# Luka140/paig_reproduction

Measured on AMD Instinct MI355X. Metric: video-seqs/sec (train step) spring_color B=100 @ 1/2/4/8 MI355X, higher is better.
Workload: dtype fp32; 1 GPU; spring_color PhysicsNet train step (get_batch gather+fwd+loss+bwd+allreduce+RMSprop), B=100/rank, 32x32x3, seq_len 50 (4 in / 6 pred / 40 extrap); global_batch=100, seq_len=50, parallelism=dp1, conv_math=split, split_graph=False, optimizer_in_graph=True, byte_targets=True, dataset_seqs=800

## Files before the change

### include/paig_hip.h

```cpp
#ifndef PAIG_HIP_H
#define PAIG_HIP_H
#include <stddef.h>

#ifdef __cplusplus
extern "C" {
#endif

#define PAIG_ABI_VERSION 9
const char* paig_last_error(void);
int paig_abi_version(void);
int paig_f16_range_status(int clear);

int paig_conv2d_fwd(const float* in, long long in_fs, int in_grp, long long in_gs, float* out, long long out_fs,
                    const float* aux, long long aux_fs, const float* w, const float* bias, int F, int Cin, int Cout,
                    int H, int W, int ks, int flags, void* stream);
#define PAIG_XMAX_SLOTS 2048
int paig_conv2d_fwd_ex(const float* in, long long in_fs, int in_grp, long long in_gs, float* out, long long out_fs,
                       const float* aux, long long aux_fs, const float* w, const float* bias, int F, int Cin,
                       int Cout, int H, int W, int ks, int flags, float* xmax, int xmax_n, void* stream);
int paig_conv2d_fwd_pw(const float* in, long long in_fs, int in_grp, long long in_gs, float* out, long long out_fs,
                       const float* aux, long long aux_fs, const float* w, const float* bias, int F, int Cin,
                       int Cout, int H, int W, int ks, int flags, float* xmax, int xmax_n, float* pool_out,
                       long long pool_fs, const void* wprep, void* stream);
int paig_conv2d_fwd_pwc(const float* in, long long in_fs, int in_grp, long long in_gs, float* out, long long out_fs,
                        const float* aux, long long aux_fs, const float* w, const float* bias, int F, int Cin,
                        int Cout, int H, int W, int ks, int flags, float* xmax, int xmax_n, float* pool_out,
                        long long pool_fs, unsigned char* pool_code, long long pool_code_fs, const void* wprep,
                        void* stream);
long long paig_conv_wprep_size(int cin, int cout, int ks);
int paig_conv_wprep(int n, const float* const* w, const int* cin, const int* cout, const int* ks, const int* dg,
                    void* const* out, void* stream);
int paig_conv_wprep_defer(int n, const float* const* w, const int* cin, const int* cout, const int* ks, const int* dg,
                          void* const* out, void* stream);
int paig_conv_wprep_flush(void* stream);
int paig_debug_fwd_block_cap(int cap);
int paig_conv2d_mfma_supported(int what, int Cin, int Cout, int H, int W, int ks, int flags);
int paig_conv2d_wgrad(const float* x, long long x_fs, int x_grp, long long x_gs, const float* dy, long long dy_fs,
                      float* slab, int nblk_max, int* nblk_out, int F, int Cin, int Cout, int H, int W, int ks,
                      int flags, void* stream);
int paig_conv2d_wgrad_ex(const float* x, long long x_fs, int x_grp, long long x_gs, const float* dy, long long dy_fs,
                         float* slab, int nblk_max, int* nblk_out, int F, int Cin, int Cout, int H, int W, int ks,
                         int flags, const float* xmax, int xmax_n, void* stream);
int paig_conv2d_bwd_supported(int Cin, int Cout, int H, int W, int ks, int flags);
int paig_conv2d_bwd(const float* x, long long x_fs, int x_grp, long long x_gs, const float* dy, long long dy_fs,
                    float* dx, long long dx_fs, const float* aux, long long aux_fs, const float* w, float* slab,
                    int nblk_max, int* nblk_out, int F, int Cin, int Cout, int H, int W, int ks, int flags,
                    const float* xmax, int xmax_n, const float* dpool, long long dpool_fs,
                    const unsigned char* pcode, long long pcode_fs, const void* wprep, void* stream);

size_t paig_unet_workspace(int net, int F, int H, int K, int math);
// ... 49 lines not shown
int paig_mask_softmax_bwd(const float* logits, const float* x, long long x_fs, int x_grp, long long x_gs,
                          const float* masks, const float* dobjs, float* dlogits, int F, int K, int C, int H, int W,
                          int flags, void* stream);
int paig_head_mask_blocks(int F, int H, int W);
int paig_head_mask_fwd(const float* x12, const float* w, const float* b, const float* x, long long x_fs, int x_grp,
                       long long x_gs, float* masks, float* objs, int F, int K, int H, int W, void* stream);
int paig_head_mask_bwd(const float* x12, const float* w, const float* b, const float* x, long long x_fs, int x_grp,
                       long long x_gs, const float* masks, const float* dobjs, float* dx12, float* slab, int F, int K,
                       int H, int W, void* stream);
int paig_head_mask_fwd_ex(const float* xl, const float* w, const float* b, const float* x, long long x_fs, int x_grp,
                          long long x_gs, float* masks, float* objs, float* pobjs, int F, int K, int CI, int H, int W,
                          int flags, void* stream);
int paig_head_mask_bwd_ex(const float* xl, const float* w, const float* b, const float* x, long long x_fs, int x_grp,
                          long long x_gs, const float* masks, const float* dobjs, float* dxl, float* slab, int F, int K,
                          int CI, int H, int W, int flags, void* stream);
int paig_pos_head_fwd(const float* h3, float* pos, int N, int K, float half, void* stream);
int paig_pos_head_bwd(const float* h3, const float* dpos, float* dh3, int N, int K, float half, void* stream);

size_t paig_gemm_workspace(int M, int N, int K);
int paig_gemm_defer_epilogue(int on);
int paig_gemm_flush(void* stream);
int paig_gemm(int ta, int tb, int M, int N, int K, float alpha, const float* A, long long lda, const float* B,
              long long ldb, float beta, float* C, long long ldc, const float* bias, int act, int auxm,
              const float* aux, long long ldaux, float* rowsum, float* ws, size_t ws_floats, void* stream);
int paig_gemm_ex(int ta, int tb, int M, int N, int K, float alpha, const float* A, long long lda, const float* B,
                 long long ldb, float beta, float* C, long long ldc, const float* bias, int act, int auxm,
                 const float* aux, long long ldaux, float* rowsum, float* ws, size_t ws_floats, int math,
                 void* stream);
size_t paig_gemm_parts_size(int M, int N, int K, int math);
int paig_gemm_parts(int ta, int tb, int M, int N, int K, const float* A, long long lda, const float* B,
                    long long ldb, float* part, size_t part_floats, int math, void* stream);
size_t paig_colsum_workspace(int M, int N);
int paig_colsum(const float* X, int M, int N, long long ld, float* out, int accumulate, float* ws, void* stream);
int paig_slab_reduce(const float* slab, int nblk, long long ld, int len, float* out, int accumulate, void* stream);
int paig_slab_reduce_multi(int ntask, const float* const* src, const int* nblk, const int* len, float* const* dst,
                           int accumulate, void* stream);
int paig_axpby(const float* x, float* y, long long n, float a, float b, void* stream);

int paig_vfn_fwd(const float* W1, const float* b1, const float* W2, const float* b2, float* hout, float* y,
                 float* ypost, int P, void* stream);
int paig_vfn_bwd_blocks(int P);
int paig_vfn_bwd(const float* d, const float* y, int sig, const float* h, const float* W2, float* dW1, float* db1,
                 float* dW2, float* db2, float* part, int P, void* stream);
// ... 159 lines not shown
```

### paig_reproduction_amd/_lib.py

```python
import ctypes
import os

import torch

_HERE = os.path.dirname(os.path.abspath(__file__))
LIB_PATH = os.path.join(_HERE, "libpaig_hip.so")
XMAX_SLOTS = 2048

AB_PATH = os.environ.get("PAIG_AB_LIB")
ABI_VERSION = 9

P = ctypes.c_void_p
I = ctypes.c_int
LL = ctypes.c_longlong
F32 = ctypes.c_float
F64 = ctypes.c_double
SZ = ctypes.c_size_t

SIGNATURES = {
    "paig_last_error": (ctypes.c_char_p, []),
    "paig_abi_version": (I, []),
    "paig_f16_range_status": (I, [I]),
    "paig_conv2d_fwd": (I, [P, LL, I, LL, P, LL, P, LL, P, P, I, I, I, I, I, I, I, P]),
    "paig_conv2d_wgrad": (I, [P, LL, I, LL, P, LL, P, I, P, I, I, I, I, I, I, I, P]),
    "paig_conv2d_fwd_ex": (I, [P, LL, I, LL, P, LL, P, LL, P, P, I, I, I, I, I, I, I, P, I, P]),
    "paig_conv2d_fwd_pw": (I, [P, LL, I, LL, P, LL, P, LL, P, P, I, I, I, I, I, I, I, P, I, P, LL, P, P]),
    "paig_conv_wprep_size": (LL, [I, I, I]),
    "paig_conv_wprep": (I, [I, P, P, P, P, P, P, P]),
    "paig_conv_wprep_defer": (I, [I, P, P, P, P, P, P, P]),
    "paig_conv_wprep_flush": (I, [P]),
    "paig_conv2d_wgrad_ex": (I, [P, LL, I, LL, P, LL, P, I, P, I, I, I, I, I, I, I, P, I, P]),
    "paig_conv2d_wgrad_pf": (I, [P, LL, I, LL, P, LL, P, LL, P, LL, P, I, P, I, I, I, I, I, I, I, P, I, P]),
    "paig_conv2d_mfma_supported": (I, [I, I, I, I, I, I, I]),
    "paig_debug_fwd_block_cap": (I, [I]),
    "paig_conv2d_bwd_supported": (I, [I, I, I, I, I, I]),
    "paig_conv2d_bwd": (I, [P, LL, I, LL, P, LL, P, LL, P, LL, P, P, I, P, I, I, I, I, I, I, I, P, I, P, LL, P, LL,
                            P, P]),
    "paig_conv2d_fwd_pwc": (I, [P, LL, I, LL, P, LL, P, LL, P, P, I, I, I, I, I, I, I, P, I, P, LL, P, LL, P, P]),
    "paig_gather_u8_f32": (I, [P, P, P, I, LL, P]),
    "paig_gather_u8_f32_ex": (I, [P, P, P, I, LL, LL, P, P]),
    "paig_velmlp_fwd": (I, [P, I, I, I, I, P, P, P, P, P, P, P, P, P, P, P]),
    "paig_velmlp_vfn_fwd": (I, [P, I, I, I, I, P, P, P, P, P, P, P, P, P, P, I, P, P, P, P, P, P, P, P, P]),
    "paig_velmlp_bwd_blocks": (I, [I]),
    "paig_velmlp_slab_len": (I, [I]),
    "paig_velmlp_bwd": (I, [P, P, P, P, P, P, P, P, P, I, I, P]),
    "paig_head_fwd": (I, [P, P, P, P, P, I, I, I, F32, P]),
    "paig_dense_tail_fwd": (I, [P, I, P, P, P, P, P, P, P, P, P, P, I, I, I, F32, P]),
    "paig_head_l2_bwd": (I, [P, P, P, P, P, P, I, I, I, F32, P, P, I, I, I, I, P, P, P, I, P, P, P, P, P, P, P, P, P,
                             P, P, P]),
# ... 17 lines not shown
    "paig_unet_query": (I, [I, I, I]),
    "paig_unet_fwd_ex": (I, [I, I, I, I, I, I, P, LL, I, LL, P, P, P, P, P, P, SZ, P, P, P]),
    "paig_unet_bwd_ex": (I, [I, I, I, I, I, I, P, LL, I, LL, P, P, P, P, I, P, P, P, P, P, P, SZ, P, P, P]),
    "paig_maxpool2_fwd": (I, [P, LL, P, LL, I, I, I, I, P]),
    "paig_maxpool2_fwd_codes": (I, [P, LL, P, LL, P, LL, I, I, I, I, P]),
    "paig_maxpool2_bwd_relu": (I, [P, LL, P, LL, P, LL, I, I, I, I, P]),
    "paig_upsample2_fwd": (I, [P, LL, P, LL, I, I, I, I, I, I, P]),
    "paig_upsample2_bwd": (I, [P, LL, P, LL, P, LL, I, I, I, I, I, I, I, P]),
    "paig_mask_softmax_fwd": (I, [P, P, LL, I, LL, P, P, P, I, I, I, I, I, P]),
    "paig_mask_softmax_bwd": (I, [P, P, LL, I, LL, P, P, P, I, I, I, I, I, I, P]),
    "paig_head_mask_blocks": (I, [I, I, I]),
    "paig_head_mask_fwd": (I, [P, P, P, P, LL, I, LL, P, P, I, I, I, I, P]),
    "paig_head_mask_bwd": (I, [P, P, P, P, LL, I, LL, P, P, P, P, I, I, I, I, P]),
    "paig_head_mask_fwd_ex": (I, [P, P, P, P, LL, I, LL, P, P, P, I, I, I, I, I, I, P]),
    "paig_head_mask_bwd_ex": (I, [P, P, P, P, LL, I, LL, P, P, P, P, I, I, I, I, I, I, P]),
    "paig_pos_head_fwd": (I, [P, P, I, I, F32, P]),
    "paig_pos_head_bwd": (I, [P, P, P, I, I, F32, P]),
    "paig_gemm_workspace": (SZ, [I, I, I]),
    "paig_gemm_parts_size": (SZ, [I, I, I, I]),
    "paig_gemm_parts": (I, [I, I, I, I, I, P, LL, P, LL, P, SZ, I, P]),
    "paig_gemm_defer_epilogue": (I, [I]),
    "paig_gemm_flush": (I, [P]),
    "paig_gemm": (I, [I, I, I, I, I, F32, P, LL, P, LL, F32, P, LL, P, I, I, P, LL, P, P, SZ, P]),
    "paig_gemm_ex": (I, [I, I, I, I, I, F32, P, LL, P, LL, F32, P, LL, P, I, I, P, LL, P, P, SZ, I, P]),
    "paig_colsum_workspace": (SZ, [I, I]),
    "paig_colsum": (I, [P, I, I, LL, P, I, P, P]),
    "paig_slab_reduce": (I, [P, I, LL, I, P, I, P]),
    "paig_slab_reduce_multi": (I, [I, P, P, P, P, I, P]),
    "paig_axpby": (I, [P, P, LL, F32, F32, P]),
    "paig_vfn_fwd": (I, [P, P, P, P, P, P, P, I, P]),
# ... 28 lines not shown
    "paig_loss_bwd": (I, [P, P, P, F32, P, P, I, I, I, I, P]),
    "paig_frame_sse": (I, [P, LL, I, LL, P, LL, I, LL, P, I, I, P]),
    "paig_frame_sse_bwd": (I, [P, LL, I, LL, P, LL, I, LL, P, P, I, I, P]),
    "paig_synth_integrate": (I, [I, P, P, LL, I, I, I, F64, F64, F64, F64, F64, P, P, P]),
    "paig_synth_raster": (I, [P, P, LL, I, I, I, F64, P, P, P]),
    "paig_rmsprop_f32": (I, [P, P, P, LL, F32, F32, F32, P]),
    "paig_rmsprop_f64": (I, [P, P, P, LL, F64, F64, F64, P]),
    "paig_rmsprop_mixed": (I, [P, P, P, LL, P, P, P, LL, F64, F64, F64, P]),
    "paig_adam_f32": (I, [P, P, P, P, LL, F32, F32, F32, F32, F32, F32, P]),
    "paig_adam_f64": (I, [P, P, P, P, LL, F64, F64, F64, F64, F64, F64, P]),
    "paig_sgd_f32": (I, [P, P, P, LL, F32, F32, I, P]),
    "paig_sgd_f64": (I, [P, P, P, LL, F64, F64, I, P]),
}

_QUERY = {"paig_last_error", "paig_abi_version", "paig_f16_range_status", "paig_conv2d_mfma_supported",
          "paig_debug_fwd_block_cap",
          "paig_conv2d_bwd_supported", "paig_velmlp_bwd_blocks",
          "paig_velmlp_slab_len", "paig_head_bwd_blocks", "paig_head_l2_bwd_blocks", "paig_head_mask_blocks", "paig_conv_wprep_size", "paig_gemm_workspace", "paig_colsum_workspace",
          "paig_gemm_parts_size", "paig_gemm_parts", "paig_unet_workspace", "paig_unet_workspace_ex",
          "paig_unet_buffer", "paig_unet_query", "paig_localiser_workspace",
          "paig_velmlp_rollout_bwd_workspace",
          "paig_vfn_bwd_blocks", "paig_rollout_bwd_blocks", "paig_decoder_bwd_blocks", "paig_decoder_slab_len",
          "paig_decoder_bwd_scratch"}


class PaigError(RuntimeError):
    pass


class _Lib:
    def __init__(self, path=LIB_PATH):
# ... 61 lines not shown
```

### paig_reproduction_amd/csrc/conv_split.hip

```cpp
#include "split_common.h"

#ifndef PAIG_FWD_AUXP
#define PAIG_FWD_AUXP 1
#endif

namespace {


constexpr bool sfwd_sla(bool UPS, int PM, int H, int W, int ups_bytes, int lo_bytes) {
  return UPS && PM == 0 && H * W >= 4096 && ups_bytes <= lo_bytes;
}
constexpr int sfwd_lds(int CIN, int H, int W, int KS, bool UPS, int PM, int tpxm, int ntb) {
  const int CC = rup(CIN, 8) / 8, PS = CC % 2 == 0 ? CC + 1 : CC;
  const int NS = ceil_div(KS * KS * CC, 4);
  const int FPT = H * W <= tpxm ? tpxm / (H * W) : 1;
  const int RT = H * W <= tpxm ? H : rows_fit(H, W, tpxm);
  const int TWPX = W + 2 * (KS / 2);
  const int RP = W == 8 ? to_mod16(TWPX * PS, 8) : TWPX * PS;
  const int img = FPT * (RT + KS - 1) * RP * 8, wimg = NS * ntb * 64 * 8;
  const int ups = UPS ? up_window_floats(CIN, FPT, RT, W) * 4 : 0;
  return (img + wimg) * 2 * (PM == 2 ? 1 : 2) + (sfwd_sla(UPS, PM, H, W, ups, img * 2) ? 0 : ups);
}
constexpr int sfwd_vgprs(int CIN, int H, int W, int KS, bool UPS, int tpxm, int ntb) {
  const int CC = rup(CIN, 8) / 8, NS = ceil_div(KS * KS * CC, 4);
// ... 1323 lines not shown
  int blk0[WPREP_MAX + 1];
  int n;
};
constexpr int WPREP_T = 256;

__device__ __forceinline__ int wprep_hdr_entries(int cout) { return (cout + 15) / 16 * 16 * 4 / 16; }

#ifndef PAIG_WPREP_S
#define PAIG_WPREP_S 8
#endif
constexpr int WPREP_S = PAIG_WPREP_S;
__device__ __forceinline__ void conv_wprep_body(const WPrepJobs& jobs, int bid) {
  int q = 0;
  while (q + 1 < jobs.n && bid >= jobs.blk0[q + 1]) ++q;
  const WPrepJob jb = jobs.j[q];
  if (jb.dg == 2) {
    __shared__ float T[32][33];
    const int bl = bid - jobs.blk0[q], tx = (bl % ((jb.cin + 31) / 32)) * 32,
              ty = (bl / ((jb.cin + 31) / 32)) * 32, c = threadIdx.x & 31, r = threadIdx.x >> 5;
    for (int y = r; y < 32; y += WPREP_T / 32)
      if (ty + y < jb.cout && tx + c < jb.cin) T[y][c] = jb.w[(long long)(ty + y) * jb.cin + tx + c];
    __syncthreads();
    float* o = reinterpret_cast<float*>(jb.out);
    for (int y = r; y < 32; y += WPREP_T / 32)
      if (tx + y < jb.cin && ty + c < jb.cout) o[(long long)(tx + y) * jb.cout + ty + c] = T[c][y];
    return;
  }
  const int KK = jb.ks * jb.ks, CC = (jb.cin + 7) / 8, KC = KK * CC, NTT = (jb.cout + 15) / 16, NS = (KC + 3) / 4;
  const int NSC = (NS + WPREP_S - 1) / WPREP_S;
  const int bl = bid - jobs.blk0[q], nt = bl / NSC, s0 = (bl % NSC) * WPREP_S;
  const int tid = threadIdx.x;
  auto wv = [&](int kc, int j, int co) {
    float v = 0.f;
    if (kc < KC && co < jb.cout) {
      const int tap = kc / CC, ci = (kc % CC) * 8 + j;
      if (ci < jb.cin) v = jb.dg ? jb.w[(ci * jb.cout + co) * KK + (KK - 1 - tap)] : jb.w[(co * jb.cin + ci) * KK + tap];
    }
    return v;
  };
  __shared__ float red[WPREP_T];
  __shared__ int ex[16];
  const int cl = tid & 15, co = nt * 16 + cl;
  float m = 0.f;
#pragma unroll 8
  for (int i = tid >> 4; i < KC * 8; i += WPREP_T / 16) m = fmaxf(m, fabsf(wv(i >> 3, i & 7, co)));
  red[tid] = m;
  __syncthreads();
  if (tid < 16) {
    float mm = 0.f;
    for (int r = 0; r < WPREP_T / 16; ++r) mm = fmaxf(mm, red[r * 16 + tid]);
    ex[tid] = f16_scale_exp_v(mm);
    if (s0 == 0) reinterpret_cast<int*>(jb.out)[nt * 16 + tid] = ex[tid];
  }
  __syncthreads();
  const int HDR = wprep_hdr_entries(jb.cout), ENT = NS * NTT * 64;
  short* img = reinterpret_cast<short*>(jb.out + HDR);
// ... 27 lines not shown

WPrepJobs g_wpend{};
int g_wpend_blocks = 0;
int wprep_build(WPrepJobs& jobs, int n, const float* const* w, const int* cin, const int* cout, const int* ks,
                const int* dg, void* const* out, int* blocks_out) {
  jobs = WPrepJobs{};
  jobs.n = n;
  int blocks = 0;
  for (int q = 0; q < n; ++q) {
    PAIG_REQUIRE(w[q] && out[q] && cin[q] > 0 && cout[q] > 0 && ks[q] > 0, "conv_wprep: job %d", q);
    PAIG_REQUIRE(((uintptr_t)out[q] & 15) == 0, "conv_wprep: job %d output not 16-byte aligned", q);
    jobs.j[q] = WPrepJob{w[q], static_cast<s16x8*>(out[q]), cin[q], cout[q], ks[q], dg[q]};
    jobs.blk0[q] = blocks;
    if (dg[q] == 2) {
      blocks += (cin[q] + 31) / 32 * ((cout[q] + 31) / 32);
      continue;
    }
    const int NS = (ks[q] * ks[q] * ((cin[q] + 7) / 8) + 3) / 4;
    blocks += (cout[q] + 15) / 16 * ((NS + WPREP_S - 1) / WPREP_S);
  }
  jobs.blk0[n] = blocks;
  *blocks_out = blocks;
  return 0;
}
int wprep_flush(hipStream_t st) {
  if (!g_wpend_blocks) return 0;
  const int nb = g_wpend_blocks;
  g_wpend_blocks = 0;
  hipLaunchKernelGGL(conv_wprep_k, dim3(nb), dim3(WPREP_T), 0, st, g_wpend);
  PAIG_CHECK_LAUNCH();
// ... 275 lines not shown
}

extern "C" {

int paig_debug_fwd_block_cap(int cap) {
  const int prev = g_fwd_block_cap;
  g_fwd_block_cap = cap > 0 ? cap : 0;
  return prev;
}

long long paig_conv_wprep_size(int cin, int cout, int ks) {
  const int KC = ks * ks * ((cin + 7) / 8), NS = (KC + 3) / 4, NTT = (cout + 15) / 16;
  return 2ll * NS * NTT * 64 * 8 + (long long)NTT * 16 * 2;
}

int paig_conv_wprep(int n, const float* const* w, const int* cin, const int* cout, const int* ks, const int* dg,
                    void* const* out, void* stream) {
  if (int rc = wprep_flush((hipStream_t)stream)) return rc;
  for (int b = 0; b < n; b += WPREP_MAX) {
    WPrepJobs jobs;
    int blocks = 0;
    const int m = n - b < WPREP_MAX ? n - b : WPREP_MAX;
    if (int rc = wprep_build(jobs, m, w + b, cin + b, cout + b, ks + b, dg + b, out + b, &blocks)) return rc;
    hipLaunchKernelGGL(conv_wprep_k, dim3(blocks), dim3(WPREP_T), 0, (hipStream_t)stream, jobs);
    PAIG_CHECK_LAUNCH();
  }
  return 0;
}

int paig_conv_wprep_defer(int n, const float* const* w, const int* cin, const int* cout, const int* ks, const int* dg,
// ... 15 lines not shown
```

### paig_reproduction_amd/csrc/gemm.hip

```cpp
#include "common.h"

#include <algorithm>
#include <cstdlib>

namespace {

constexpr int BM = 64, BN = 64, BK = 32;
constexpr int LDRK = BK + 2;
constexpr int LDKR = 64 + 16;
constexpr int IMG = (BK * LDKR > 64 * LDRK ? BK * LDKR : 64 * LDRK);

typedef float f32x4 __attribute__((ext_vector_type(4)));

__device__ __attribute__((aligned(16))) float zero16[4];

template <bool KCONTIG>
struct Tile {
  f32x4 v[2];
  __device__ __forceinline__ void load(const float* __restrict__ p, long long ld, int r0, int k0, int R, int K,
                                       bool vec, int tid) {
#pragma unroll
    for (int e = 0; e < 2; ++e) {
      int r, k;
      if (KCONTIG) { r = (tid >> 3) + 32 * e; k = (tid & 7) * 4; }
// ... 839 lines not shown
    if (tile == 1) PAIG_W((gemm_split_w_k<TA, TB, PM_, true, 64, 256>)); \
    else if (tile == 2) PAIG_W((gemm_split_w_k<TA, TB, PM_, true, 256, 64>)); \
    else PAIG_S(PM_);                                                   \
  } while (0)
  if (math == 1) PAIG_S(1);
  else if (math == 2) PAIG_S(2);
  else if (math == 3) PAIG_SW(3);
  else if (math == 4) PAIG_SW(4);
  else if (math == 5) PAIG_S(5);
  else if (math == 6) PAIG_SW(6);
  else PAIG_L((gemm_k<TA, TB>));
#undef PAIG_SW
#undef PAIG_S
#undef PAIG_W
#undef PAIG_L
}

}

static PendEpi make_epi(int M, int N, int S, const float* part, float* C, long long ldc, float beta, const float* bias,
                        int act, int auxm, const float* aux, long long ldaux, const float* rowpart, float* rowsum) {
  const bool v4 = N % 4 == 0 && vec_ok(C, ldc) && (!bias || (uintptr_t)bias % 16 == 0) &&
                  (!aux || auxm == AUX_NONE || vec_ok(aux, ldaux)) && (uintptr_t)part % 16 == 0 &&
                  (long long)S * M * N < (1ll << 31) && (long long)M * ldc < (1ll << 31) &&
                  (long long)M * ldaux < (1ll << 31) &&
                  (long long)M * N >= (1 << 19);
  return PendEpi{M, N, S, part, C, ldc, beta, bias, act, auxm, aux, ldaux, rowpart, rowsum, v4 ? 1 : 0};
}
static void launch_epi(const PendEpi& e, hipStream_t st) {
  long long n_el = (e.v4 ? (long long)e.M * e.N / 4 : (long long)e.M * e.N) + (e.rowsum ? e.M : 0);
// ... 129 lines not shown
  else PAIG_G(false, false);
#undef PAIG_G
  PAIG_CHECK_LAUNCH();
  if (S > 1) {
    const PendEpi e = make_epi(M, N, S, part, C, ldc, beta, bias, act, auxm, aux, ldaux, rowpart, rowsum);
    if (defer) {
      g_pend = e;
    } else {
      launch_epi(e, st);
      PAIG_CHECK_LAUNCH();
    }
  }
  return 0;
}

}

PAIG_F16_RANGE_ACCESSOR(paig_f16_range_gemm)
```

### paig_reproduction_amd/csrc/unet_ops.hip

```cpp
#include "common.h"

#define PAIG_MAX_SLAB_TASKS 32

namespace {

template <typename I>
__global__ void maxpool_fwd_k(FView x, FViewW y, int F, int C, int H, int W) {
  const int Ho = H / 2, Wo = W / 2;
  const I n = (I)F * C * Ho * Wo;
  for (I i = blockIdx.x * (I)blockDim.x + threadIdx.x; i < n; i += (I)gridDim.x * blockDim.x) {
    int j = i % Wo;
    I t = i / Wo;
    int ii = t % Ho;
    t /= Ho;
    int c = t % C;
    int f = (int)(t / C);
    const float* xp = x.frame(f) + ((long long)c * H + 2 * ii) * W + 2 * j;
    float m = xp[0];
    float v = xp[1];
    if (v > m || v != v) m = v;
    v = xp[W];
    if (v > m || v != v) m = v;
    v = xp[W + 1];
    if (v > m || v != v) m = v;
// ... 541 lines not shown
            pa[k][c].x += o[1];
            pa[k][c].y += o[2];
            pa[k][c].y += o[3];
          }
      }
    }
#pragma unroll
    for (int k = 0; k < K; ++k)
#pragma unroll
      for (int c = 0; c < 3; ++c)
        *reinterpret_cast<float2*>(pobjs + ((long long)k * F + f) * 3 * HW4 + (long long)c * HW4 + py * W2 + 2 * u) =
            make_float2(pa[k][c].x * 0.25f, pa[k][c].y * 0.25f);
  }
}

template <int K, int CI, bool RELU, bool POOL>
__global__ void __launch_bounds__(256) head_mask_bwd_k(const float* __restrict__ xl, const float* __restrict__ w,
                                                       const float* __restrict__ b, FView x,
                                                       const float* __restrict__ masks, const float* __restrict__ dobjs,
                                                       float* __restrict__ dxl, float* __restrict__ slab, int F, int H,
                                                       int W) {
  constexpr int NW = K * CI + K;
  const int HW = H * W, W2 = W / 2, HW4 = (H / 2) * W2;
  const int DHW = POOL ? HW4 : HW;
  const int Q = HW / 4;
  const long long n = (long long)F * Q;
  float acc[NW];
#pragma unroll
  for (int t = 0; t < NW; ++t) acc[t] = 0.f;
  for (long long i = blockIdx.x * (long long)blockDim.x + threadIdx.x; i < n; i += (long long)gridDim.x * blockDim.x) {
    const int p = (int)(i % Q) * 4;
    const int f = (int)(i / Q);
    const int pq = POOL ? ((p / W) >> 1) * W2 + ((p % W) >> 1) : p;
    m4 hv[CI];
#pragma unroll
    for (int c = 0; c < CI; ++c) hv[c] = *reinterpret_cast<const m4*>(xl + ((long long)f * CI + c) * HW + p);
    const float* xp = x.frame(f);
    m4 xv[3];
#pragma unroll
    for (int c = 0; c < 3; ++c) xv[c] = *reinterpret_cast<const m4*>(xp + c * HW + p);
    m4 dm[K], mk[K];
    m4 dot = m4{0.f, 0.f, 0.f, 0.f};
#pragma unroll
    for (int k = 0; k < K; ++k) {
      m4 a = m4{0.f, 0.f, 0.f, 0.f};
#pragma unroll
      for (int c = 0; c < 3; ++c) {
        const float* dp = dobjs + ((long long)k * F + f) * 3 * DHW + (long long)c * DHW + pq;
        m4 d;
        if constexpr (POOL) {
          const float2 dq = *reinterpret_cast<const float2*>(dp);
          d = m4{dq.x, dq.x, dq.y, dq.y} * 0.25f;
        } else {
          d = *reinterpret_cast<const m4*>(dp);
        }
#pragma unroll
        for (int j = 0; j < 4; ++j) a[j] = fmaf(d[j], xv[c][j], a[j]);
      }
      dm[k] = a;
      mk[k] = *reinterpret_cast<const m4*>(masks + ((long long)f * (K + 1) + k) * HW + p);
#pragma unroll
      for (int j = 0; j < 4; ++j) dot[j] = fmaf(mk[k][j], a[j], dot[j]);
// ... 394 lines not shown
                       logits, FView{x, x_fs, x_gs, x_grp}, masks, dobjs, dlogits, F, K, C, H, W, flags);
  PAIG_CHECK_LAUNCH();
  return 0;
}

static bool head_mask_ok(const void* a, const void* b, const void* c, const void* d, const void* e, long long x_fs,
                         long long x_gs, int K, int H, int W) {
  return (H * W) % 4 == 0 && (K == 2 || K == 3) && x_fs % 4 == 0 && x_gs % 4 == 0 &&
         ((uintptr_t)a | (uintptr_t)b | (uintptr_t)c | (uintptr_t)d | (uintptr_t)e) % 16 == 0;
}
static bool head_mask_kind(int CI, int flags, int H, int W, const void* pobjs) {
  if (CI == 8 && flags == 1) return true;
  return CI == 16 && flags == 2 && H % 2 == 0 && W % 4 == 0 && ((uintptr_t)pobjs % 8) == 0;
}

int paig_head_mask_blocks(int F, int H, int W) {
  const long long n = (long long)F * H * W / 4;
  long long g = (n + 255) / 256;
  return (int)(g < 1 ? 1 : (g > 1024 ? 1024 : g));
}

int paig_head_mask_fwd_ex(const float* xl, const float* w, const float* b, const float* x, long long x_fs, int x_grp,
                          long long x_gs, float* masks, float* objs, float* pobjs, int F, int K, int CI, int H, int W,
                          int flags, void* stream) {
  if (F <= 0) return 0;
  PAIG_REQUIRE(head_mask_ok(xl, x, masks, objs, nullptr, x_fs, x_gs, K, H, W),
               "head_mask_fwd: needs K in {2,3}, H*W %% 4 == 0 and 16-byte aligned buffers (K=%d H=%d W=%d)", K, H, W);
  PAIG_REQUIRE(head_mask_kind(CI, flags, H, W, pobjs) && (!(flags & 2) || pobjs),
               "head_mask_fwd: (CI=%d, flags=%d) is neither the ShallowUNet head (8, 1) nor the UNet's (16, 2)", CI,
               flags);
  const FView xv{x, x_fs, x_gs, x_grp};
  hipStream_t st = (hipStream_t)stream;
  if (flags & 2) {
    const dim3 g(grid_for((long long)F * (H / 2) * (W / 4)));
// ... 19 lines not shown
               flags);
  const dim3 g(paig_head_mask_blocks(F, H, W));
  const FView xv{x, x_fs, x_gs, x_grp};
  hipStream_t st = (hipStream_t)stream;
  if (flags & 2) {
    if (K == 2) hipLaunchKernelGGL((head_mask_bwd_k<2, 16, false, true>), g, dim3(256), 0, st, xl, w, b, xv, masks, dobjs, dxl, slab, F, H, W);
    else hipLaunchKernelGGL((head_mask_bwd_k<3, 16, false, true>), g, dim3(256), 0, st, xl, w, b, xv, masks, dobjs, dxl, slab, F, H, W);
  } else {
    if (K == 2) hipLaunchKernelGGL((head_mask_bwd_k<2, 8, true, false>), g, dim3(256), 0, st, xl, w, b, xv, masks, dobjs, dxl, slab, F, H, W);
    else hipLaunchKernelGGL((head_mask_bwd_k<3, 8, true, false>), g, dim3(256), 0, st, xl, w, b, xv, masks, dobjs, dxl, slab, F, H, W);
  }
  PAIG_CHECK_LAUNCH();
  return 0;
}

int paig_head_mask_fwd(const float* x12, const float* w, const float* b, const float* x, long long x_fs, int x_grp,
                       long long x_gs, float* masks, float* objs, int F, int K, int H, int W, void* stream) {
  return paig_head_mask_fwd_ex(x12, w, b, x, x_fs, x_grp, x_gs, masks, objs, nullptr, F, K, 8, H, W, 1, stream);
}

int paig_head_mask_bwd(const float* x12, const float* w, const float* b, const float* x, long long x_fs, int x_grp,
                       long long x_gs, const float* masks, const float* dobjs, float* dx12, float* slab, int F, int K,
                       int H, int W, void* stream) {
  return paig_head_mask_bwd_ex(x12, w, b, x, x_fs, x_grp, x_gs, masks, dobjs, dx12, slab, F, K, 8, H, W, 1, stream);
}

int paig_pos_head_fwd(const float* h3, float* pos, int N, int K, float half, void* stream) {
  hipLaunchKernelGGL(pos_head_fwd_k, dim3(grid_for(N * K * 2)), dim3(256), 0, (hipStream_t)stream, h3, pos, N, K, half);
  PAIG_CHECK_LAUNCH();
  return 0;
// ... 89 lines not shown
```

### paig_reproduction_amd/engine.py

```python
import ctypes
import os

import torch

from ._lib import PaigError, lib, ptr, stream_handle, require_device



class Layout:

    def __init__(self, model, B, T, frames=None, net=None):
        self.B, self.T = B, T
        self.K = model.n_objs
        self.D = model.coord_units // 2
        self.H = model.conv_input_shape[1]
        self.h = self.H // 2
        self.ins, self.pred = model.input_steps, model.pred_steps
        self.Te = self.ins + self.pred
        self.R = model.pred_steps + model.extrap_steps
        if frames is None:
            assert T == model.seq_len, f"input has {T} frames, model expects seq_len={model.seq_len}"
            self.F = B * self.Te
        else:
            self.F = frames
# ... 161 lines not shown
        gW, gb = self.g(name + ".weight"), self.g(name + ".bias")
        n_ws = ws.numel()
        if defer_epi:
            self.L.paig_gemm_defer_epilogue(1)
        with self._p("gemm_wgrad:" + name, 2 * rows * O * I, 4 * (rows * O + rows * I + O * I + O)):
            self.L.paig_gemm_ex(1, 0, O, I, rows, 1.0, ptr(dy), O, ptr(x), I, 0.0, ptr(gW), I, None, 0, 0, None, 0,
                                ptr(gb), ptr(ws), n_ws, self.gemm_math(self.WGRAD), st)
        if need_dx:
            with self._p("gemm_dgrad:" + name, 2 * rows * O * I, 4 * (rows * O + O * I + (2 if auxm else 1) * rows * I)):
                self.L.paig_gemm_ex(0, 0, rows, I, O, 1.0, ptr(dy), O, ptr(W), I, 0.0, ptr(dx), I, None, 0, auxm,
                                    ptr(aux), I, None, ptr(ws), n_ws, self.gemm_math(self.DGRAD), st)

    def dense_tail(self):
        return self.gemm_math(self.FWD) == 6 and os.environ.get("PAIG_DENSE_TAIL", "1") != "0"

    def workspace_floats(self, lay):
        K, F, B = lay.K, lay.F, lay.B
        n1 = lay.l1_in
        need = [self.L.paig_gemm_workspace(K * F, 200, n1), self.L.paig_gemm_workspace(K * F, 200, 200),
                self.L.paig_gemm_workspace(200, n1, K * F), self.L.paig_gemm_workspace(K * F, n1, 200), self.L.paig_gemm_workspace(200, 200, K * F),
                self.L.paig_gemm_workspace(2, 200, K * F), self.L.paig_gemm_workspace(100, 100, K * B),
                self.L.paig_gemm_workspace(200, 200, K * F) + self.L.paig_gemm_workspace(200, n1, K * F),
                self.L.paig_gemm_workspace(K * B, 100, 100), 1 << 16,
                self.L.paig_gemm_parts_size(K * F, 200, n1, self.gemm_math(self.FWD))]
        return int(max(need))

    def forward(self, x, need_saved=True):
        require_device(x)
        model = self.model
        model._flat.ensure()
# ... 194 lines not shown
        Bs = [self.p(lay.prefix + f"c{c + 1}.bias") for c in range(lay.nconv)]
        wp = {}
        wpf = wpd = None
        if cm == self.CONV_MATH["split"]:
            flags |= 8
            jobs = []
            for c, W_ in enumerate(Ws):
                cout, cin, ks = W_.shape[0], W_.shape[1], W_.shape[-1]
                jobs.append((c, 0, W_, cin, cout, ks))
                if c > 0:
                    jobs.append((c, 1, W_, cout, cin, ks))
            sizes = [int(L.paig_conv_wprep_size(j[3], j[4], j[5])) for j in jobs]
            if self.dense_tail():
                jobs.append((-1, 2, self.p("encoder.l2.weight"), 200, 200, 1))
                sizes.append(2 * 200 * 200)
            buf = torch.empty(sum(-(-n // 8) * 8 for n in sizes), dtype=torch.int16, device=dev)
            outs, off = [], 0
            for j, n in zip(jobs, sizes):
                wp[(j[0], j[1])] = buf.data_ptr() + 2 * off
                outs.append(wp[(j[0], j[1])])
                off += -(-n // 8) * 8
            n = len(jobs)
            wprep = L.paig_conv_wprep_defer if os.environ.get("PAIG_WPREP_MERGE", "1") != "0" else L.paig_conv_wprep
            wprep(n, (ctypes.c_void_p * n)(*[ptr(j[2]) for j in jobs]),
                  (ctypes.c_int * n)(*[j[3] for j in jobs]), (ctypes.c_int * n)(*[j[4] for j in jobs]),
                  (ctypes.c_int * n)(*[j[5] for j in jobs]), (ctypes.c_int * n)(*[j[1] for j in jobs]),
                  (ctypes.c_void_p * n)(*outs), st)
            S["wprep_buf"] = buf
            wpf = _parr([wp[(c, 0)] for c in range(lay.nconv)])
            wpd = _parr([wp.get((c, 1), 0) for c in range(lay.nconv)])
# ... 271 lines not shown
        elif vel is not None and vel[6] is not None:
            dXv, dpos0, Bv, Tev, Sv, altv, vfn2 = vel
            L.paig_head_bwd_vel_vfn2(ptr(S["h2"]), ptr(S["h3"]), ptr(denc), ptr(self.p("encoder.l3.weight")),
                                     ptr(dh2), ptr(hslab), F, K, 200, float(H / 2), ptr(dXv), ptr(dpos0), Bv, Tev,
                                     Sv, altv, *vfn2, st)
        elif vel is not None:
            dXv, dpos0, Bv, Tev, Sv, altv, _ = vel
            L.paig_head_bwd_vel(ptr(S["h2"]), ptr(S["h3"]), ptr(denc), ptr(self.p("encoder.l3.weight")), ptr(dh2),
                                ptr(hslab), F, K, 200, float(H / 2), ptr(dXv), ptr(dpos0), Bv, Tev, Sv, altv, st)
        else:
            L.paig_head_bwd(ptr(S["h2"]), ptr(S["h3"]), ptr(denc), ptr(self.p("encoder.l3.weight")), ptr(dh2),
                            ptr(hslab), F, K, 200, float(H / 2), st)
        g3 = self.g("encoder.l3.weight")
        assert self.g("encoder.l3.bias").data_ptr() == g3.data_ptr() + 400 * 4, "l3 grads not contiguous"
        S["extra_slabs"].append((hslab, hblk, 402, g3))
        dobjs = _empty(K * F * lay.l1_in, dev)
        merge = os.environ.get("PAIG_GEMM_EPI_MERGE", "1") != "0" and not self.probe
        w2 = int(L.paig_gemm_workspace(200, 200, K * F)) if merge else 0
        self.linear_bwd(S["h1"], dh2, K * F, "encoder.l2", dh1, S["h1"], 1, st, ws, need_dx=not fused_l2,
                        defer_epi=merge)
        self.linear_bwd(S["l1_x"], dh1, K * F, "encoder.l1", dobjs, None, 0, st, ws[w2:] if merge else ws,
                        defer_epi=merge)
        if merge:
            L.paig_gemm_flush(st)
        if hook and self.bucket_hook is not None:
            self.bucket_hook()

        acts = S["acts"]
        if S.get("head_fused"):
            hn, c = lay.prefix + lay.head_name, lay.head_ci
            dXl = self._unet_grad(S, lay.head_buf, F * c * HW)
            nb = L.paig_head_mask_blocks(F, H, H)
            nw = K * c + K
            hs = _empty(nb * nw, dev)
            L.paig_head_mask_bwd_ex(ptr(acts["head"]), ptr(self.p(hn + ".weight")), ptr(self.p(hn + ".bias")),
                                    *x_view, ptr(S["masks"]), ptr(dobjs), ptr(dXl), ptr(hs), F, K, c, H, H,
                                    lay.head_flags, st)
            gh = self.g(hn + ".weight")
            assert self.g(hn + ".bias").data_ptr() == gh.data_ptr() + K * c * 4, "head grads not contiguous"
            S["extra_slabs"].append((hs, nb, nw, gh))
            self._unet_backward(S, None, st)
        else:
            dLG = _empty(F * K * HW, dev)
            L.paig_mask_softmax_bwd(ptr(acts["LG"]), x_view[0], x_view[1], x_view[2], x_view[3], ptr(S["masks"]),
                                    ptr(dobjs), ptr(dLG), F, K, 3, H, H,
                                    (1 if lay.lg_relu else 0) | (2 if lay.unet else 0), st)
            self._unet_backward(S, dLG, st)

    @staticmethod
    def _check_fresh(S):
        if S.get("consumed"):
            raise PaigError("a second backward through one forward (retain_graph=True) is not supported: the "
# ... 24 lines not shown
```

Measured before the change: 98840 video-seqs/s.

## Fuse encoder l1 dgrad with image-channel reduction into per-pixel mask gradient

Adds a split-fp16 MFMA kernel that computes the encoder l1 input gradient and immediately contracts it with the input frame's three color channels. This produces a per-pixel mask gradient (K*F*HW) instead of the full K*F*3*HW dobjs tensor. A new weight-prep job (kind 3) pre-packs the l1 weight into an MFMA image with per-column exponents. The head-mask backward gets a DM variant that reads the contracted gradient and skips the input-frame load and 3-channel dot. The aim is to cut the HBM write and read of the large dobjs buffer and one pass of work, at the cost of a new specialized kernel and split-precision scaling complexity.

Result: no change. 99640 video-seqs/s (median of 6 runs) (+0.8%).

```diff
diff --git a/include/paig_hip.h b/include/paig_hip.h
--- a/include/paig_hip.h
+++ b/include/paig_hip.h
@@ -28,12 +28,14 @@
                         long long pool_fs, unsigned char* pool_code, long long pool_code_fs, const void* wprep,
                         void* stream);
 long long paig_conv_wprep_size(int cin, int cout, int ks);
+long long paig_conv_wprep_size_ex(int cin, int cout, int ks, int dg);
 int paig_conv_wprep(int n, const float* const* w, const int* cin, const int* cout, const int* ks, const int* dg,
                     void* const* out, void* stream);
 int paig_conv_wprep_defer(int n, const float* const* w, const int* cin, const int* cout, const int* ks, const int* dg,
                           void* const* out, void* stream);
 int paig_conv_wprep_flush(void* stream);
 int paig_debug_fwd_block_cap(int cap);
+int paig_debug_head_mask_block_cap(int cap);
 int paig_conv2d_mfma_supported(int what, int Cin, int Cout, int H, int W, int ks, int flags);
 int paig_conv2d_wgrad(const float* x, long long x_fs, int x_grp, long long x_gs, const float* dy, long long dy_fs,
                       float* slab, int nblk_max, int* nblk_out, int F, int Cin, int Cout, int H, int W, int ks,
@@ -113,6 +115,8 @@
 int paig_head_mask_bwd_ex(const float* xl, const float* w, const float* b, const float* x, long long x_fs, int x_grp,
                           long long x_gs, const float* masks, const float* dobjs, float* dxl, float* slab, int F, int K,
                           int CI, int H, int W, int flags, void* stream);
+int paig_head_mask_bwd_dm(const float* xl, const float* w, const float* b, const float* masks, const float* dm,
+                          float* dxl, float* slab, int F, int K, int CI, int H, int W, int flags, void* stream);
 int paig_pos_head_fwd(const float* h3, float* pos, int N, int K, float half, void* stream);
 int paig_pos_head_bwd(const float* h3, const float* dpos, float* dh3, int N, int K, float half, void* stream);
 
@@ -126,6 +130,8 @@
                  long long ldb, float beta, float* C, long long ldc, const float* bias, int act, int auxm,
                  const float* aux, long long ldaux, float* rowsum, float* ws, size_t ws_floats, int math,
                  void* stream);
+int paig_l1_dgrad_dm(const float* dh1, int R, int O, const void* w1img, const float* x, long long x_fs, int x_grp,
+                     long long x_gs, int F, int HW, float* dm, void* stream);
 size_t paig_gemm_parts_size(int M, int N, int K, int math);
 int paig_gemm_parts(int ta, int tb, int M, int N, int K, const float* A, long long lda, const float* B,
                     long long ldb, float* part, size_t part_floats, int math, void* stream);
diff --git a/paig_reproduction_amd/_lib.py b/paig_reproduction_amd/_lib.py
--- a/paig_reproduction_amd/_lib.py
+++ b/paig_reproduction_amd/_lib.py
@@ -26,6 +26,7 @@
     "paig_conv2d_fwd_ex": (I, [P, LL, I, LL, P, LL, P, LL, P, P, I, I, I, I, I, I, I, P, I, P]),
     "paig_conv2d_fwd_pw": (I, [P, LL, I, LL, P, LL, P, LL, P, P, I, I, I, I, I, I, I, P, I, P, LL, P, P]),
     "paig_conv_wprep_size": (LL, [I, I, I]),
+    "paig_conv_wprep_size_ex": (LL, [I, I, I, I]),
     "paig_conv_wprep": (I, [I, P, P, P, P, P, P, P]),
     "paig_conv_wprep_defer": (I, [I, P, P, P, P, P, P, P]),
     "paig_conv_wprep_flush": (I, [P]),
@@ -33,6 +34,7 @@
     "paig_conv2d_wgrad_pf": (I, [P, LL, I, LL, P, LL, P, LL, P, LL, P, I, P, I, I, I, I, I, I, I, P, I, P]),
     "paig_conv2d_mfma_supported": (I, [I, I, I, I, I, I, I]),
     "paig_debug_fwd_block_cap": (I, [I]),
+    "paig_debug_head_mask_block_cap": (I, [I]),
     "paig_conv2d_bwd_supported": (I, [I, I, I, I, I, I]),
     "paig_conv2d_bwd": (I, [P, LL, I, LL, P, LL, P, LL, P, LL, P, P, I, P, I, I, I, I, I, I, I, P, I, P, LL, P, LL,
                             P, P]),
@@ -80,6 +82,8 @@
     "paig_head_mask_bwd": (I, [P, P, P, P, LL, I, LL, P, P, P, P, I, I, I, I, P]),
     "paig_head_mask_fwd_ex": (I, [P, P, P, P, LL, I, LL, P, P, P, I, I, I, I, I, I, P]),
     "paig_head_mask_bwd_ex": (I, [P, P, P, P, LL, I, LL, P, P, P, P, I, I, I, I, I, I, P]),
+    "paig_head_mask_bwd_dm": (I, [P, P, P, P, P, P, P, I, I, I, I, I, I, P]),
+    "paig_l1_dgrad_dm": (I, [P, I, I, P, P, LL, I, LL, I, I, P, P]),
     "paig_pos_head_fwd": (I, [P, P, I, I, F32, P]),
     "paig_pos_head_bwd": (I, [P, P, P, I, I, F32, P]),
     "paig_gemm_workspace": (SZ, [I, I, I]),
@@ -138,7 +142,7 @@
 }
 
 _QUERY = {"paig_last_error", "paig_abi_version", "paig_f16_range_status", "paig_conv2d_mfma_supported",
-          "paig_debug_fwd_block_cap",
+          "paig_debug_fwd_block_cap", "paig_debug_head_mask_block_cap", "paig_conv_wprep_size_ex",
           "paig_conv2d_bwd_supported", "paig_velmlp_bwd_blocks",
           "paig_velmlp_slab_len", "paig_head_bwd_blocks", "paig_head_l2_bwd_blocks", "paig_head_mask_blocks", "paig_conv_wprep_size", "paig_gemm_workspace", "paig_colsum_workspace",
           "paig_gemm_parts_size", "paig_gemm_parts", "paig_unet_workspace", "paig_unet_workspace_ex",
diff --git a/paig_reproduction_amd/csrc/conv_split.hip b/paig_reproduction_amd/csrc/conv_split.hip
--- a/paig_reproduction_amd/csrc/conv_split.hip
+++ b/paig_reproduction_amd/csrc/conv_split.hip
@@ -1361,6 +1361,45 @@
   int q = 0;
   while (q + 1 < jobs.n && bid >= jobs.blk0[q + 1]) ++q;
   const WPrepJob jb = jobs.j[q];
+  __shared__ float red[WPREP_T];
+  __shared__ int ex[16];
+  if (jb.dg == 3) {
+    const int O = jb.cin, HW = jb.cout, C = jb.ks, KT = (O + 31) / 32, NPT = (HW + 15) / 16;
+    const int bl = bid - jobs.blk0[q], c = bl / NPT, pt = bl % NPT, tid = threadIdx.x;
+    const long long ldw = (long long)C * HW;
+    const float* wc = jb.w + (long long)c * HW + pt * 16;
+    float m = 0.f;
+    if (pt * 16 + (tid & 15) < HW)
+#pragma unroll 4
+      for (int j = tid >> 4; j < O; j += WPREP_T / 16) m = fmaxf(m, fabsf(wc[j * ldw + (tid & 15)]));
+    red[tid] = m;
+    __syncthreads();
+    if (tid < 16) {
+      float mm = 0.f;
+      for (int r = 0; r < WPREP_T / 16; ++r) mm = fmaxf(mm, red[r * 16 + tid]);
+      ex[tid] = f16_scale_exp_v(mm);
+      reinterpret_cast<int*>(jb.out)[(c * NPT + pt) * 16 + tid] = ex[tid];
+    }
+    __syncthreads();
+    s16x8* img = reinterpret_cast<s16x8*>(reinterpret_cast<int*>(jb.out) + C * NPT * 16) +
+                 (long long)(c * NPT + pt) * KT * 128;
+    for (int t = tid; t < KT * 64; t += WPREP_T) {
+      const int kt = t >> 6, ln = t & 63, col = ln & 15, k0 = kt * 32 + 8 * (ln >> 4);
+      s16x8 h, l;
+#pragma unroll
+      for (int j = 0; j < 8; ++j) {
+        const float v = (pt * 16 + col < HW && k0 + j < O) ? wc[(k0 + j) * ldw + col] : 0.f;
+        float rm = 0.f;
+        short hs, ls;
+        split<0>(__builtin_amdgcn_ldexpf(v, ex[col]), hs, ls, rm);
+        h[j] = hs;
+        l[j] = ls;
+      }
+      img[kt * 128 + ln] = h;
+      img[kt * 128 + 64 + ln] = l;
+    }
+    return;
+  }
   if (jb.dg == 2) {
     __shared__ float T[32][33];
     const int bl = bid - jobs.blk0[q], tx = (bl % ((jb.cin + 31) / 32)) * 32,
@@ -1385,8 +1424,6 @@
     }
     return v;
   };
-  __shared__ float red[WPREP_T];
-  __shared__ int ex[16];
   const int cl = tid & 15, co = nt * 16 + cl;
   float m = 0.f;
 #pragma unroll 8
@@ -1444,6 +1481,11 @@
     jobs.blk0[q] = blocks;
     if (dg[q] == 2) {
       blocks += (cin[q] + 31) / 32 * ((cout[q] + 31) / 32);
+      continue;
+    }
+    if (dg[q] == 3) {
+      PAIG_REQUIRE(ks[q] == 3, "conv_wprep: job %d (kind 3) needs 3 image channels, got %d", q, ks[q]);
+      blocks += ks[q] * ((cout[q] + 15) / 16);
       continue;
     }
     const int NS = (ks[q] * ks[q] * ((cin[q] + 7) / 8) + 3) / 4;
@@ -1749,6 +1791,12 @@
   return 2ll * NS * NTT * 64 * 8 + (long long)NTT * 16 * 2;
 }
 
+long long paig_conv_wprep_size_ex(int cin, int cout, int ks, int dg) {
+  if (dg != 3) return paig_conv_wprep_size(cin, cout, ks);
+  const long long NPT = (cout + 15) / 16, KT = (cin + 31) / 32;
+  return ks * NPT * 16 * 2 + ks * NPT * KT * 2 * 64 * 8;
+}
+
 int paig_conv_wprep(int n, const float* const* w, const int* cin, const int* cout, const int* ks, const int* dg,
                     void* const* out, void* stream) {
   if (int rc = wprep_flush((hipStream_t)stream)) return rc;
diff --git a/paig_reproduction_amd/csrc/gemm.hip b/paig_reproduction_amd/csrc/gemm.hip
--- a/paig_reproduction_amd/csrc/gemm.hip
+++ b/paig_reproduction_amd/csrc/gemm.hip
@@ -877,6 +877,128 @@
 #undef PAIG_S
 #undef PAIG_W
 #undef PAIG_L
+}
+
+constexpr int DM_KTMAX = 7;
+constexpr int DM_PITCH = DM_KTMAX * 32 + 16;
+
+template <int MI, int KT>
+__global__ void __launch_bounds__(256)
+l1_dgrad_dm_k(const float* __restrict__ dh, int R, int O, const int* __restrict__ wexp,
+              const s16x8* __restrict__ wimg, FView x, int F, int HW, float* __restrict__ dm, int nstrip, int tpb,
+              int nepi, PendEpi pe) {
+  if ((int)blockIdx.x < nepi) {
+    splitk_epi_run(pe, blockIdx.x, nepi);
+    return;
+  }
+  constexpr int RS = 16 * MI;
+  constexpr int E = RS * KT * 8 / 256;
+  static_assert(RS * KT * 8 % 256 == 0, "strip float4s per thread");
+  __shared__ __attribute__((aligned(16))) short SA[2 * RS * DM_PITCH];
+  __shared__ float smx[4];
+  short* Ah = SA;
+  short* Al = SA + RS * DM_PITCH;
+  const int tid = threadIdx.x, lane = tid & 63, wv = tid >> 6;
+  const int total = (int)gridDim.x - nepi;
+  int lin = (int)blockIdx.x - nepi;
+  if (total % 8 == 0 && nepi % 8 == 0) lin = (lin % 8) * (total / 8) + lin / 8;
+  const int r0 = (lin % nstrip) * RS, cg = lin / nstrip;
+  const int NPT = (HW + 15) >> 4;
+
+  f32x4 v[E];
+  float m = 0.f;
+#pragma unroll
+  for (int e = 0; e < E; ++e) {
+    const int q = tid + 256 * e, row = q / (KT * 8), gk = (q % (KT * 8)) * 4, gr = r0 + row;
+    const bool ok = gr < R && gk < O;
+    v[e] = *reinterpret_cast<const f32x4*>(ok ? dh + (long long)gr * O + gk : zero16);
+    m = amax2(amax2(m, v[e][0], v[e][1]), v[e][2], v[e][3]);
+  }
+  m = wave_max_u(m);
+  if (lane == 0) smx[wv] = m;
+  __syncthreads();
+  const int ea = f16_scale_exp(fmaxf(fmaxf(smx[0], smx[1]), fmaxf(smx[2], smx[3])));
+  const float asc = __builtin_amdgcn_ldexpf(1.f, ea);
+#pragma unroll
+  for (int e = 0; e < E; ++e) {
+    const int q = tid + 256 * e, row = q / (KT * 8), k = (q % (KT * 8)) * 4;
+    const pf32x2 a = pf32x2{v[e][0], v[e][1]} * asc, b = pf32x2{v[e][2], v[e][3]} * asc;
+    const HiLo qa = split_pk(a.x, a.y), qb = split_pk(b.x, b.y);
+    *reinterpret_cast<u32x2*>(Ah + row * DM_PITCH + k) = u32x2{qa.h, qb.h};
+    *reinterpret_cast<u32x2*>(Al + row * DM_PITCH + k) = u32x2{qa.l, qb.l};
+  }
+  __syncthreads();
+
+  const int q1 = min((cg + 1) * tpb, (NPT + 3) >> 2);
+  for (int q = cg * tpb; q < q1; ++q) {
+    const int pt = q * 4 + wv;
+    if (pt >= NPT) continue;
+    f32x4 acc[MI][3];
+#pragma unroll
+    for (int i = 0; i < MI; ++i)
+#pragma unroll
+      for (int c = 0; c < 3; ++c) acc[i][c] = f32x4{0.f, 0.f, 0.f, 0.f};
+    const s16x8* wp[3];
+#pragma unroll
+    for (int c = 0; c < 3; ++c) wp[c] = wimg + (long long)(c * NPT + pt) * (KT * 2 * 64) + lane;
+    s16x8 w[2][3][2];
+#pragma unroll
+    for (int c = 0; c < 3; ++c) {
+      w[0][c][0] = wp[c][0];
+      w[0][c][1] = wp[c][64];
+    }
+#pragma unroll
+    for (int kt = 0; kt < KT; ++kt) {
+      if (kt + 1 < KT) {
+#pragma unroll
+        for (int c = 0; c < 3; ++c) {
+          w[(kt + 1) & 1][c][0] = wp[c][(kt + 1) * 128];
+          w[(kt + 1) & 1][c][1] = wp[c][(kt + 1) * 128 + 64];
+        }
+      }
+      s16x8 dhh[MI], dhl[MI];
+#pragma unroll
+      for (int i = 0; i < MI; ++i) {
+        const int o = (i * 16 + (lane & 15)) * DM_PITCH + kt * 32 + 8 * (lane >> 4);
+        dhh[i] = *reinterpret_cast<const s16x8*>(Ah + o);
+        dhl[i] = *reinterpret_cast<const s16x8*>(Al + o);
+      }
+#pragma unroll
+      for (int i = 0; i < MI; ++i)
+#pragma unroll
+        for (int c = 0; c < 3; ++c) {
+          acc[i][c] = gmma<6>(w[kt & 1][c][1], dhh[i], acc[i][c]);
+          acc[i][c] = gmma<6>(w[kt & 1][c][0], dhl[i], acc[i][c]);
+          acc[i][c] = gmma<6>(w[kt & 1][c][0], dhh[i], acc[i][c]);
+        }
+    }
+    const int pl = pt * 16 + (lane >> 4) * 4;
+    if (pl < HW) {
+      int ec[3][4];
+#pragma unroll
+      for (int c = 0; c < 3; ++c) {
+        const int4 t = *reinterpret_cast<const int4*>(wexp + c * NPT * 16 + pl);
+        ec[c][0] = t.x, ec[c][1] = t.y, ec[c][2] = t.z, ec[c][3] = t.w;
+      }
+#pragma unroll
+      for (int i = 0; i < MI; ++i) {
+        const int row = r0 + i * 16 + (lane & 15);
+        if (row < R) {
+          const float* xp = x.frame(row % F) + pl;
+          f32x4 xv[3];
+#pragma unroll
+          for (int c = 0; c < 3; ++c) xv[c] = *reinterpret_cast<const f32x4*>(xp + (long long)c * HW);
+          f32x4 o = f32x4{0.f, 0.f, 0.f, 0.f};
+#pragma unroll
+          for (int c = 0; c < 3; ++c)
+#pragma unroll
+            for (int r = 0; r < 4; ++r)
+              o[r] = fmaf(__builtin_amdgcn_ldexpf(acc[i][c][r], -(ea + ec[c][r])), xv[c][r], o[r]);
+          *reinterpret_cast<f32x4*>(dm + (long long)row * HW + pl) = o;
+        }
+      }
+    }
+  }
 }
 
 }
@@ -1036,6 +1158,49 @@
   return 0;
 }
 
+int paig_l1_dgrad_dm(const float* dh1, int R, int O, const void* w1img, const float* x, long long x_fs, int x_grp,
+                     long long x_gs, int F, int HW, float* dm, void* stream) {
+  if (R <= 0 || HW <= 0) return paig_gemm_flush(stream);
+  PAIG_REQUIRE(O > 0 && O % 4 == 0 && O <= DM_KTMAX * 32, "paig_l1_dgrad_dm: O=%d must be a multiple of 4 in 4..%d", O,
+               DM_KTMAX * 32);
+  PAIG_REQUIRE(F > 0 && R % F == 0 && HW % 4 == 0, "paig_l1_dgrad_dm: R=%d rows of F=%d frames, HW=%d", R, F, HW);
+  PAIG_REQUIRE(((uintptr_t)dh1 | (uintptr_t)w1img | (uintptr_t)x | (uintptr_t)dm) % 16 == 0 && x_fs % 4 == 0 &&
+                   x_gs % 4 == 0 && dh1 && w1img && x && dm,
+               "paig_l1_dgrad_dm: buffers must be 16-byte aligned");
+  constexpr int mi = 2, tpb = 1;
+  const int KT = cdiv(O, 32), NPT = cdiv(HW, 16), nstrip = cdiv(R, 16 * mi), ncg = cdiv(cdiv(NPT, 4), tpb);
+  const PendEpi pe = take_pending();
+  int nepi = 0;
+  if (pe.S) {
+    const long long n_el = (pe.v4 ? (long long)pe.M * pe.N / 4 : (long long)pe.M * pe.N) + (pe.rowsum ? pe.M : 0);
+    nepi = cdiv(std::min<long long>(cdiv(n_el, 256), 1024), 8) * 8;
+  }
+  const int* wexp = static_cast<const int*>(w1img);
+  const s16x8* wimg = reinterpret_cast<const s16x8*>(wexp + 3 * NPT * 16);
+  const FView xv{x, x_fs, x_gs, x_grp};
+  const dim3 grid(nepi + nstrip * ncg);
+#define PAIG_DM(MI_, KT_)                                                                                         \
+  hipLaunchKernelGGL((l1_dgrad_dm_k<MI_, KT_>), grid, dim3(256), 0, (hipStream_t)stream, dh1, R, O, wexp, wimg, xv, F, \
+                     HW, dm, nstrip, tpb, nepi, pe)
+#define PAIG_DMK(KT_) \
+  case KT_:           \
+    PAIG_DM(mi, KT_); \
+    break
+  switch (KT) {
+    PAIG_DMK(1);
+    PAIG_DMK(2);
+    PAIG_DMK(3);
+    PAIG_DMK(4);
+    PAIG_DMK(5);
+    PAIG_DMK(6);
+    PAIG_DMK(7);
+  }
+#undef PAIG_DMK
+#undef PAIG_DM
+  PAIG_CHECK_LAUNCH();
+  return 0;
+}
+
 }
 
 PAIG_F16_RANGE_ACCESSOR(paig_f16_range_gemm)
diff --git a/paig_reproduction_amd/csrc/unet_ops.hip b/paig_reproduction_amd/csrc/unet_ops.hip
--- a/paig_reproduction_amd/csrc/unet_ops.hip
+++ b/paig_reproduction_amd/csrc/unet_ops.hip
@@ -579,7 +579,7 @@
   }
 }
 
-template <int K, int CI, bool RELU, bool POOL>
+template <int K, int CI, bool RELU, bool POOL, bool DM = false>
 __global__ void __launch_bounds__(256) head_mask_bwd_k(const float* __restrict__ xl, const float* __restrict__ w,
                                                        const float* __restrict__ b, FView x,
                                                        const float* __restrict__ masks, const float* __restrict__ dobjs,
@@ -600,17 +600,20 @@
     m4 hv[CI];
 #pragma unroll
     for (int c = 0; c < CI; ++c) hv[c] = *reinterpret_cast<const m4*>(xl + ((long long)f * CI + c) * HW + p);
-    const float* xp = x.frame(f);
     m4 xv[3];
-#pragma unroll
-    for (int c = 0; c < 3; ++c) xv[c] = *reinterpret_cast<const m4*>(xp + c * HW + p);
+    if constexpr (!DM) {
+      const float* xp = x.frame(f);
+#pragma unroll
+      for (int c = 0; c < 3; ++c) xv[c] = *reinterpret_cast<const m4*>(xp + c * HW + p);
+    }
     m4 dm[K], mk[K];
     m4 dot = m4{0.f, 0.f, 0.f, 0.f};
 #pragma unroll
     for (int k = 0; k < K; ++k) {
       m4 a = m4{0.f, 0.f, 0.f, 0.f};
-#pragma unroll
-      for (int c = 0; c < 3; ++c) {
+      if constexpr (DM) a = *reinterpret_cast<const m4*>(dobjs + ((long long)k * F + f) * HW + p);
+#pragma unroll
+      for (int c = 0; c < (DM ? 0 : 3); ++c) {
         const float* dp = dobjs + ((long long)k * F + f) * 3 * DHW + (long long)c * DHW + pq;
         m4 d;
         if constexpr (POOL) {
@@ -1035,10 +1038,18 @@
   return CI == 16 && flags == 2 && H % 2 == 0 && W % 4 == 0 && ((uintptr_t)pobjs % 8) == 0;
 }
 
+static int g_head_mask_block_cap = 0;
+int paig_debug_head_mask_block_cap(int cap) {
+  const int prev = g_head_mask_block_cap;
+  g_head_mask_block_cap = cap > 0 ? cap : 0;
+  return prev;
+}
+
 int paig_head_mask_blocks(int F, int H, int W) {
   const long long n = (long long)F * H * W / 4;
   long long g = (n + 255) / 256;
-  return (int)(g < 1 ? 1 : (g > 1024 ? 1024 : g));
+  const int cap = g_head_mask_block_cap ? g_head_mask_block_cap : 1024;
+  return (int)(g < 1 ? 1 : (g > cap ? cap : g));
 }
 
 int paig_head_mask_fwd_ex(const float* xl, const float* w, const float* b, const float* x, long long x_fs, int x_grp,
@@ -1088,6 +1099,22 @@
   return 0;
 }
 
+int paig_head_mask_bwd_dm(const float* xl, const float* w, const float* b, const float* masks, const float* dm,
+                          float* dxl, float* slab, int F, int K, int CI, int H, int W, int flags, void* stream) {
+  if (F <= 0) return 0;
+  PAIG_REQUIRE(head_mask_ok(xl, nullptr, masks, dm, dxl, 0, 0, K, H, W),
+               "head_mask_bwd_dm: needs K in {2,3}, H*W %% 4 == 0 and 16-byte aligned buffers (K=%d H=%d W=%d)", K, H, W);
+  PAIG_REQUIRE(CI == 8 && flags == 1, "head_mask_bwd_dm: (CI=%d, flags=%d) is not the ShallowUNet head (8, 1)", CI,
+               flags);
+  const dim3 g(paig_head_mask_blocks(F, H, W));
+  const FView xv{nullptr, 0, 0, 0};
+  hipStream_t st = (hipStream_t)stream;
+  if (K == 2) hipLaunchKernelGGL((head_mask_bwd_k<2, 8, true, false, true>), g, dim3(256), 0, st, xl, w, b, xv, masks, dm, dxl, slab, F, H, W);
+  else hipLaunchKernelGGL((head_mask_bwd_k<3, 8, true, false, true>), g, dim3(256), 0, st, xl, w, b, xv, masks, dm, dxl, slab, F, H, W);
+  PAIG_CHECK_LAUNCH();
+  return 0;
+}
+
 int paig_head_mask_fwd(const float* x12, const float* w, const float* b, const float* x, long long x_fs, int x_grp,
                        long long x_gs, float* masks, float* objs, int F, int K, int H, int W, void* stream) {
   return paig_head_mask_fwd_ex(x12, w, b, x, x_fs, x_grp, x_gs, masks, objs, nullptr, F, K, 8, H, W, 1, stream);
diff --git a/paig_reproduction_amd/engine.py b/paig_reproduction_amd/engine.py
--- a/paig_reproduction_amd/engine.py
+++ b/paig_reproduction_amd/engine.py
@@ -199,6 +199,12 @@
     def dense_tail(self):
         return self.gemm_math(self.FWD) == 6 and os.environ.get("PAIG_DENSE_TAIL", "1") != "0"
 
+    def l1_dgrad_fused(self, lay):
+        W1 = self.p("encoder.l1.weight")
+        return (self.gemm_math(self.DGRAD) == 6 and self.conv_flags() == self.CONV_MATH["split"] and lay.fuse_head
+                and not lay.unet and lay.head_flags == 1 and W1.shape[1] == 3 * lay.HW and W1.shape[0] % 4 == 0
+                and W1.shape[0] <= 224 and os.environ.get("PAIG_L1_DGRAD_FUSED", "1") != "0")
+
     def workspace_floats(self, lay):
         K, F, B = lay.K, lay.F, lay.B
         n1 = lay.l1_in
@@ -423,6 +429,10 @@
             if self.dense_tail():
                 jobs.append((-1, 2, self.p("encoder.l2.weight"), 200, 200, 1))
                 sizes.append(2 * 200 * 200)
+            if fuse_head and self.l1_dgrad_fused(lay):
+                o1 = self.p("encoder.l1.weight").shape[0]
+                jobs.append((-2, 3, self.p("encoder.l1.weight"), o1, lay.HW, 3))
+                sizes.append(int(L.paig_conv_wprep_size_ex(o1, lay.HW, 3, 3)))
             buf = torch.empty(sum(-(-n // 8) * 8 for n in sizes), dtype=torch.int16, device=dev)
             outs, off = [], 0
             for j, n in zip(jobs, sizes):
@@ -724,13 +734,19 @@
         g3 = self.g("encoder.l3.weight")
         assert self.g("encoder.l3.bias").data_ptr() == g3.data_ptr() + 400 * 4, "l3 grads not contiguous"
         S["extra_slabs"].append((hslab, hblk, 402, g3))
-        dobjs = _empty(K * F * lay.l1_in, dev)
+        w1img = S.get("wprep", {}).get((-2, 3)) if S.get("head_fused") else None
+        dobjs = _empty(K * F * (HW if w1img is not None else lay.l1_in), dev)
         merge = os.environ.get("PAIG_GEMM_EPI_MERGE", "1") != "0" and not self.probe
         w2 = int(L.paig_gemm_workspace(200, 200, K * F)) if merge else 0
         self.linear_bwd(S["h1"], dh2, K * F, "encoder.l2", dh1, S["h1"], 1, st, ws, need_dx=not fused_l2,
                         defer_epi=merge)
         self.linear_bwd(S["l1_x"], dh1, K * F, "encoder.l1", dobjs, None, 0, st, ws[w2:] if merge else ws,
-                        defer_epi=merge)
+                        need_dx=w1img is None, defer_epi=merge)
+        if w1img is not None:
+            O1 = self.p("encoder.l1.weight").shape[0]
+            with self._p("gemm_dgrad:encoder.l1", 2 * K * F * O1 * 3 * HW + 6 * K * F * HW,
+                         4 * (K * F * O1 + O1 * 3 * HW + F * 3 * HW + K * F * HW)):
+                L.paig_l1_dgrad_dm(ptr(dh1), K * F, O1, w1img, *x_view, F, HW, ptr(dobjs), st)
         if merge:
             L.paig_gemm_flush(st)
         if hook and self.bucket_hook is not None:
@@ -743,9 +759,14 @@
             nb = L.paig_head_mask_blocks(F, H, H)
             nw = K * c + K
             hs = _empty(nb * nw, dev)
-            L.paig_head_mask_bwd_ex(ptr(acts["head"]), ptr(self.p(hn + ".weight")), ptr(self.p(hn + ".bias")),
-                                    *x_view, ptr(S["masks"]), ptr(dobjs), ptr(dXl), ptr(hs), F, K, c, H, H,
-                                    lay.head_flags, st)
+            if w1img is not None:
+                L.paig_head_mask_bwd_dm(ptr(acts["head"]), ptr(self.p(hn + ".weight")), ptr(self.p(hn + ".bias")),
+                                        ptr(S["masks"]), ptr(dobjs), ptr(dXl), ptr(hs), F, K, c, H, H,
+                                        lay.head_flags, st)
+            else:
+                L.paig_head_mask_bwd_ex(ptr(acts["head"]), ptr(self.p(hn + ".weight")), ptr(self.p(hn + ".bias")),
+                                        *x_view, ptr(S["masks"]), ptr(dobjs), ptr(dXl), ptr(hs), F, K, c, H, H,
+                                        lay.head_flags, st)
             gh = self.g(hn + ".weight")
             assert self.g(hn + ".bias").data_ptr() == gh.data_ptr() + K * c * 4, "head grads not contiguous"
             S["extra_slabs"].append((hs, nb, nw, gh))
```
